# dusk-network/dusk-blindbidproof

Measured on AMD Instinct MI355X. Metric: blind-bid proofs/sec, higher is better.
Workload: dtype u32

## Files before the change

__graft_entry__.py:

```python
import os
import shutil
import subprocess
import sys

ROOT = os.path.dirname(os.path.abspath(__file__))
PKG = os.path.join(ROOT, "dusk_blindbidproof_amd")
CSRC = os.path.join(PKG, "csrc")
LIB = os.path.join(PKG, "libbbp_hip.so")
ORACLE_SO = os.path.join(ROOT, "oracle", "_build", "libbbp_oracle.so")
HOSTCHECK_SO = os.path.join(ROOT, "tests", "_build", "libhostcheck.so")
DEVCHECK_SO = {"chain": os.path.join(ROOT, "tests", "_build", "libbbp_devcheck.so"),
               "nochain": os.path.join(ROOT, "tests", "_build", "libbbp_devcheck_nochain.so")}
DEVCHECK_DEFS = {"chain": [], "nochain": ["-DBBP_FE_NO_CHAIN"]}


def _newer(target, sources):
    if not os.path.exists(target):
        return True
    t = os.path.getmtime(target)
    return any(os.path.getmtime(s) > t for s in sources)


def _run(cmd):
    print("+", " ".join(cmd), flush=True)
# ... 177 lines not shown
VERIFY_PLAN_SAN_BIN = os.path.join(ROOT, "tests", "_build", "verify_plan_san")


def build_verify_plan_san(force=False):
    src = os.path.join(ROOT, "tests", "verify_plan_san.cpp")
    if force or _newer(VERIFY_PLAN_SAN_BIN, [src, os.path.join(ROOT, "tests", "host_check.cpp")] + _csrc_files((".h", ".inc"))):
        os.makedirs(os.path.dirname(VERIFY_PLAN_SAN_BIN), exist_ok=True)
        _run(["g++", "-O1", "-g", "-std=c++17", "-fsanitize=address,undefined", "-fno-sanitize-recover=all", "-o", VERIFY_PLAN_SAN_BIN, src])
    return VERIFY_PLAN_SAN_BIN


BATCH_LAYOUT_SAN_BIN = os.path.join(ROOT, "tests", "_build", "batch_layout_san")


def build_batch_layout_san(force=False):
    src = os.path.join(ROOT, "tests", "batch_layout_san.cpp")
    if force or _newer(BATCH_LAYOUT_SAN_BIN, [src, os.path.join(ROOT, "tests", "host_check.cpp")] + _csrc_files((".h", ".inc"))):
        os.makedirs(os.path.dirname(BATCH_LAYOUT_SAN_BIN), exist_ok=True)
        _run(["g++", "-O1", "-g", "-std=c++17", "-fsanitize=address,undefined", "-fno-sanitize-recover=all", "-o", BATCH_LAYOUT_SAN_BIN, src])
    return BATCH_LAYOUT_SAN_BIN


HEDGE_SAN_BIN = os.path.join(ROOT, "tests", "_build", "hedge_san")


def build_hedge_san(force=False):
    src = os.path.join(ROOT, "tests", "hedge_san.cpp")
    if force or _newer(HEDGE_SAN_BIN, [src] + _csrc_files((".h", ".inc"))):
        os.makedirs(os.path.dirname(HEDGE_SAN_BIN), exist_ok=True)
        _run(["g++", "-O1", "-g", "-std=c++17", "-fsanitize=address,undefined", "-fno-sanitize-recover=all", "-o", HEDGE_SAN_BIN, src])
    return HEDGE_SAN_BIN


SECRET_MAP_BIN = os.path.join(ROOT, "tests", "_build", "secret_map_check")
SECRET_WIPE_SAN_BIN = os.path.join(ROOT, "tests", "_build", "secret_wipe_san")


def build_secret_map_check(force=False):
    src = os.path.join(ROOT, "tests", "secret_map_check.cpp")
    if force or _newer(SECRET_MAP_BIN, [src] + _csrc_files((".h", ".inc"))):
        os.makedirs(os.path.dirname(SECRET_MAP_BIN), exist_ok=True)
        _run(["g++", "-O1", "-g", "-std=c++17", "-fsanitize=address,undefined", "-fno-sanitize-recover=all", "-o", SECRET_MAP_BIN, src])
    return SECRET_MAP_BIN


ROUND_SELECT_BIN = os.path.join(ROOT, "tests", "_build", "round_select_check")


def build_round_select_check(force=False):
    src = os.path.join(ROOT, "tests", "round_select_check.cpp")
    if force or _newer(ROUND_SELECT_BIN, [src] + _csrc_files((".h", ".inc")) + [os.path.join(ROOT, "include", "bbp.h")]):
        os.makedirs(os.path.dirname(ROUND_SELECT_BIN), exist_ok=True)
        _run(["g++", "-O1", "-g", "-std=c++17", "-fsanitize=address,undefined", "-fno-sanitize-recover=all", "-o", ROUND_SELECT_BIN, src])
    return ROUND_SELECT_BIN


ROUND_BEST_BIN = os.path.join(ROOT, "tests", "_build", "round_best_check")


def build_round_best_check(force=False):
    src = os.path.join(ROOT, "tests", "round_best_check.cpp")
    if force or _newer(ROUND_BEST_BIN, [src] + _csrc_files((".h", ".inc")) + [os.path.join(ROOT, "include", "bbp.h")]):
        os.makedirs(os.path.dirname(ROUND_BEST_BIN), exist_ok=True)
        _run(["g++", "-O1", "-g", "-std=c++17", "-fsanitize=address,undefined", "-fno-sanitize-recover=all", "-o", ROUND_BEST_BIN, src])
    return ROUND_BEST_BIN

# ... 105 lines not shown
        flags = ["-O1", "-g", "-fsanitize=thread"] if tsan else ["-O1"]
        _run(["g++"] + flags + ["-std=c++17", "-pthread", "-o", out] + srcs)
    return out


COMBINER_ROUNDS_BIN = {False: os.path.join(ROOT, "tests", "_build", "combiner_rounds"), True: os.path.join(ROOT, "tests", "_build", "combiner_rounds_tsan")}


def build_combiner_rounds(tsan=False, force=False):
    out = COMBINER_ROUNDS_BIN[bool(tsan)]
    srcs = [os.path.join(ROOT, "tests", "combiner_rounds.cpp"), os.path.join(CSRC, "submit.cpp")]
    if force or _newer(out, srcs + [os.path.join(CSRC, "submit.h")]):
        os.makedirs(os.path.dirname(out), exist_ok=True)
        flags = ["-O1", "-g", "-fsanitize=thread"] if tsan else ["-O1"]
        _run(["g++"] + flags + ["-std=c++17", "-pthread", "-o", out] + srcs)
    return out


def build():
    build_hip()
    build_server()
    build_stub_engine()
    build_oracle()
    build_hostcheck()
    build_sortcheck()
    build_roundcheck()
    build_round_select_check()
    build_round_best_check()
    build_round_best_distinct_check()
    build_rounds_best_check()
    build_rounds_best_distinct_check()
    build_round_standing_check()
    build_standings_check()
    build_devcheck_all()
    sys.path.insert(0, ROOT)
    import dusk_blindbidproof_amd


def smoke():
    sys.path.insert(0, ROOT)
    import dusk_blindbidproof_amd as bbp
    from tests import smoke_case

    smoke_case.run(bbp)


if __name__ == "__main__":
    build()
```

dusk_blindbidproof_amd/csrc/msm.hip:

```cpp
#include "context.h"

namespace bbp {

#ifndef BBP_FOLD_PRIO
#define BBP_FOLD_PRIO 2
#endif
#ifndef BBP_MSM_WAVES
#define BBP_MSM_WAVES 2
#endif
#ifndef BBP_MSM_WAVES_MAX
#define BBP_MSM_WAVES_MAX 2
#endif

#ifdef BBP_MSM_PROF
__device__ unsigned long long g_msm_prof[8];
#define MSM_PROF_BEGIN() unsigned long long prof_t = wall_clock64()
#define MSM_PROF_MARK(i)                                                    \
    if (tid == 0) {                                                         \
        unsigned long long now_ = wall_clock64();                           \
        atomicAdd(&g_msm_prof[i], now_ - prof_t);                           \
        prof_t = now_;                                                      \
    }
#else
#define MSM_PROF_BEGIN()
// ... 466 lines not shown
        ge acc = ge_identity();
        u32 ent_cur = sorted[c0];
        u32 ent_nxt = (c0 + 1 < c1) ? sorted[c0 + 1] : 0u;
        row_regs row = load_row(ptable, ent_cur, fault);
        for (u32 e = c0; e < c1; e++) {
            if (e == kend) {
                *dest = acc;
                acc = ge_identity();
                do { k++; kend = cursor[k]; } while (kend == e);
                dest = &bsum[k - 1];
            }
            const row_regs cur = row;
            const bool neg = ent_cur >> 31;
            ent_cur = ent_nxt;
            if (e + 1 < c1) row = load_row(ptable, ent_cur, fault);
            if (e + 2 < c1) ent_nxt = sorted[e + 2];
            acc = ge_madd_row(acc, cur, neg);
        }
        *dest = acc;
    }
#endif
#ifdef BBP_MSM_PROF
    if (tid == 0) atomicAdd(&g_msm_prof[6], clock64() - clk0);
#endif
    MSM_PROF_MARK(2);
    __threadfence_block();
    __syncthreads();
    MSM_PROF_MARK(3);
#ifdef BBP_ACC_PERSIST
  }
#endif
}

template <int MODE>
__global__ __launch_bounds__(MSM_T) void k_msm_fold(const u32* __restrict__ cursor_all, ge* __restrict__ bsum_all, const ge* __restrict__ psum_all,
                                                     ge* __restrict__ out, const u32* __restrict__ n_active) {
    constexpr int K = msm_geom<MODE>::K, G = K / MSM_T;
    __shared__ u32 cursor[K + 1];
    __shared__ u32 xch[GE_WORDS];
    const int tid = threadIdx.x;
    if (n_active && blockIdx.x >= *n_active) return;
    __builtin_amdgcn_s_setprio(BBP_FOLD_PRIO);
    const size_t msm = blockIdx.x;
    {
        const u32* cur_in = cursor_all + msm * (size_t)(K + 1);
        for (int k = tid; k <= K; k += MSM_T) cursor[k] = cur_in[k];
    }
    __syncthreads();
    const u32 E = cursor[K];
    ge* bsum = bsum_all + msm * (size_t)K;
    const ge* psum = psum_all + msm * (size_t)ACC_T;
#ifdef BBP_KO_FOLD
    if (MODE != 1) { if (tid == 0) out[msm] = bsum[0]; }
    else if (tid < FOLD_CLS) out[msm * FOLD_CLS + tid] = bsum[tid];
    return;
#endif
    for (u32 ch = tid; ch < (u32)ACC_T; ch += MSM_T) {
        const u32 c0 = (u32)(((u64)ch * E) / ACC_T), c1 = (u32)(((u64)(ch + 1) * E) / ACC_T);
        if (c0 >= c1) continue;
        u32 lo = 1, hi = K;
        while (lo < hi) {
            u32 mid = (lo + hi) >> 1;
            if (cursor[mid] > c0) hi = mid; else lo = mid + 1;
        }
        const u32 k_first = lo;
        const bool inside = cursor[lo - 1] < c0;
        const bool last_of_run = inside && !(c1 < E && c1 > cursor[k_first - 1] && c1 < cursor[k_first]);
        if (last_of_run) {
            ge part = psum[ch];
            for (int u = (int)ch - 1; u >= 0; u--) {
                const u32 cu = (u32)(((u64)u * E) / ACC_T), cu1 = (u32)(((u64)(u + 1) * E) / ACC_T);
                if (cu <= cursor[k_first - 1]) break;
                if (cu1 > cu) ge_add_nc(part, part, psum[u]);
            }
            ge head = bsum[k_first - 1];
            ge_add_nc(head, head, part);
            bsum[k_first - 1] = head;
        }
    }
    __threadfence_block();
    __syncthreads();

    ge running = ge_identity(), total = ge_identity();
    if constexpr (G == 1) {
        if (cursor[tid + 1] != cursor[tid]) running = bsum[tid];
        total = running;
    } else {
#pragma unroll 1
        for (int r = G; r >= 1; r--) {
            const u32 k = tid * G + r;
            if (cursor[k] != cursor[k - 1]) running = ge_add(running, bsum[k - 1]);
            total = ge_add(total, running);
        }
    }

    if constexpr (MODE != 1) {
        const int lane = tid & 63, wave = tid >> 6;
#pragma unroll 1
        for (int d = 1; d < 64; d <<= 1) {
            ge other = ge_shfl_down(running, d);
            if (lane + d < 64) running = ge_add(running, other);
        }
        if (MSM_T > 64) {
            if (tid == 64) xch_put(xch, running);
            __syncthreads();
            if (wave == 0) {
                ge other = xch_get(xch);
                ge_add_nc(running, running, other);
            }
        }
        ge x = total;
        if (tid >= 1) {
            ge s = running;
            constexpr int LOG_G = G == 1 ? 0 : G == 2 ? 1 : G == 4 ? 2 : G == 8 ? 3 : G == 16 ? 4 : -1;
            static_assert(LOG_G >= 0, "buckets per fold lane must be a power of two up to 16");
            for (int i = 0; i < LOG_G; i++) ge_dbl_nc(s, s);
            ge_add_nc(x, x, s);
        }
#pragma unroll 1
        for (int d = 32; d >= 1; d >>= 1) {
            ge other = ge_shfl_down(x, d);
            if (lane < d) x = ge_add(x, other);
        }
        if (MSM_T > 64) {
            __syncthreads();
            if (tid == 64) xch_put(xch, x);
            __syncthreads();
        }
        if (tid == 0) {
            if (MSM_T > 64) {
                ge other = xch_get(xch);
                ge_add_nc(x, x, other);
            }
            ge other;
            ge_dbl_nc(x, x);
            other = ge_neg(running);
            ge_add_nc(x, x, other);
            out[msm] = x;
        }
    } else {
        constexpr int LPC = FOLD_M / G, LOG_G2 = G == 32 ? 5 : 6;
        static_assert(G == 32 || G == 64, "class reduction written for 4 or 2 lanes per class");
        const int q = tid & (LPC - 1);
        ge suf = running;
        for (int d = 1; d < LPC; d++) {
            ge other = ge_shfl_down(running, d);
            if (q + d < LPC) ge_add_nc(suf, suf, other);
        }
        ge x = total;
        if (q >= 1) {
            ge sg = suf;
            for (int i = 0; i < LOG_G2; i++) ge_dbl_nc(sg, sg);
            ge_add_nc(x, x, sg);
        }
        ge accq = x;
        for (int d = 1; d < LPC; d++) {
            ge other = ge_shfl_down(x, d);
            if (q == 0) ge_add_nc(accq, accq, other);
        }
        if (q == 0) {
            ge_dbl_nc(accq, accq);
            ge other = ge_neg(suf);
            ge_add_nc(accq, accq, other);
            out[msm * FOLD_CLS + (tid / LPC)] = accq;
        }
    }
}

constexpr int FOLD2_L = 32;
constexpr int FOLD2_G = MSM_K / FOLD2_L;
constexpr int FOLD2_LOG_G = 5;
static_assert(FOLD2_G == 32 && ACC_T % FOLD2_L == 0, "fold geometry");

__device__ __forceinline__ ge ge_shfl_down32(const ge& p, int d) {
    ge r;
    const u32* w = reinterpret_cast<const u32*>(&p);
    u32* o = reinterpret_cast<u32*>(&r);
#pragma unroll
    for (int i = 0; i < GE_WORDS; i++) o[i] = (u32)__shfl_down((int)w[i], d, 32);
    return r;
}

__device__ __forceinline__ ge ge_add_t2d(const ge& p, const fe& p2d, const ge& q) {
    fe a = fe_mul(fe_sub(p.Y, p.X), fe_sub(q.Y, q.X));
    fe b = fe_mul(fe_add(p.Y, p.X), fe_add(q.Y, q.X));
    fe c = fe_mul(p2d, q.T);
    fe zz = fe_mul(p.Z, q.Z);
    fe d = fe_add(zz, zz);
    fe e = fe_sub(b, a), f = fe_sub(d, c), g = fe_add(d, c), h = fe_add(b, a);
    ge r;
    r.X = fe_mul(e, f);
    r.Y = fe_mul(g, h);
    r.Z = fe_mul(g, f);
    r.T = fe_mul(e, h);
    return r;
}

__device__ __forceinline__ void park_put(u32* park, int tid, const ge& p) {
    const u32* w = reinterpret_cast<const u32*>(&p);
#pragma unroll
    for (int i = 0; i < GE_WORDS; i++) park[i * 64 + tid] = w[i];
}

__device__ __forceinline__ ge park_get(const u32* park, int tid) {
    ge p;
    u32* w = reinterpret_cast<u32*>(&p);
#pragma unroll
    for (int i = 0; i < GE_WORDS; i++) w[i] = park[i * 64 + tid];
    return p;
}

__device__ __forceinline__ ge ld_ge(const ge* p) {
    ge r;
    const uint4* s = reinterpret_cast<const uint4*>(p);
    u32* o = reinterpret_cast<u32*>(&r);
#pragma unroll
    for (int i = 0; i < GE_WORDS / 4; i++) {
        const uint4 v = s[i];
        o[4 * i] = v.x, o[4 * i + 1] = v.y, o[4 * i + 2] = v.z, o[4 * i + 3] = v.w;
    }
    return r;
}

#ifndef BBP_FOLD_WAVES
#define BBP_FOLD_WAVES 2
#endif
__global__ __launch_bounds__(64) __attribute__((amdgpu_waves_per_eu(BBP_FOLD_WAVES, BBP_FOLD_WAVES))) void k_msm_fold_half(const u32* __restrict__ cursor_all, ge* __restrict__ bsum_all, const ge* __restrict__ psum_all,
                                                       ge* __restrict__ out, u32 n_work, const u32* __restrict__ n_active) {
    constexpr int K = MSM_K, G = FOLD2_G;
    __shared__ u32 cursor2[2][K + 1];
    __shared__ u32 park[GE_WORDS * 64];
    const int tid = threadIdx.x, half = tid >> 5, l = tid & 31;
    const u32 n_tot = n_active ? min(*n_active, n_work) : n_work;
    if (2u * blockIdx.x >= n_tot) return;
    __builtin_amdgcn_s_setprio(BBP_FOLD_PRIO);
    const size_t msm = 2 * (size_t)blockIdx.x + half;
    const bool valid = msm < n_tot;
    u32* cursor = cursor2[half];
    {
        const u32* cur_in = cursor_all + msm * (size_t)(K + 1);
        for (int k = l; k <= K; k += FOLD2_L) cursor[k] = valid ? cur_in[k] : 0u;
    }
    __syncthreads();
    const u32 E = cursor[K];
    ge* bsum = bsum_all + (valid ? msm : 0) * (size_t)K;
    const ge* psum = psum_all + (valid ? msm : 0) * (size_t)ACC_T;
#pragma unroll 1
    for (u32 ch = l; ch < (u32)ACC_T; ch += FOLD2_L) {
        const u32 c0 = (u32)(((u64)ch * E) / ACC_T), c1 = (u32)(((u64)(ch + 1) * E) / ACC_T);
        bool last_of_run = false;
        u32 k_first = 1;
        if (c0 < c1) {
            u32 lo = 1, hi = K;
            while (lo < hi) {
// ... 319 lines not shown
```

dusk_blindbidproof_amd/csrc/prover.hip:

```cpp
#define BBP_KECCAK_WAVE 1
#include <string.h>

#include <functional>

#include "batch.h"
#include "hosthash.h"
#include "keccak_wave.h"
#include "scalarmul.h"
#include "witness.h"

namespace bbp {

#define BBP_THIN_PRIO() __builtin_amdgcn_s_setprio(3)
#ifndef BBP_LANE_KERNEL
#define BBP_LANE_KERNEL __launch_bounds__(64)
#endif


__device__ __forceinline__ void sc_to_bytes32(uint8_t* o, const sc& s) { sc_tobytes(o, s); }
__device__ __forceinline__ void words_to_bytes32(uint8_t* o, const u32* w) {
#pragma unroll
    for (int i = 0; i < 8; i++) {
        o[4 * i] = (uint8_t)w[i];
        o[4 * i + 1] = (uint8_t)(w[i] >> 8);
// ... 848 lines not shown
}

__global__ __launch_bounds__(64) __attribute__((amdgpu_waves_per_eu(2, 3))) void k_tail_tables(u32 count, const ge* __restrict__ pts, ge* __restrict__ tab) {
    BBP_THIN_PRIO();
    u32 t = blockIdx.x * blockDim.x + threadIdx.x;
    if (t >= count) return;
    ge P = pts[t];
    ge* T = tab + (size_t)t * TAIL_TAB;
#pragma unroll 1
    for (int k = 0; k < TAIL_PIECES; k++) {
        ge cur = P;
        T[8 * k] = P;
#pragma unroll 1
        for (int i = 1; i < 8; i++) {
            cur = ge_add(cur, P);
            T[8 * k + i] = cur;
        }
        if (k < TAIL_PIECES - 1) {
#pragma unroll 1
            for (int i = 0; i < TAIL_PIECE_BITS; i++) P = ge_dbl(P);
        }
    }
}

__global__ void k_tail_init(u32 B, sc* __restrict__ g_all, sc* __restrict__ h_all) {
    BBP_THIN_PRIO();
    u32 t = blockIdx.x * blockDim.x + threadIdx.x;
    if (t >= B * FOLD_CLS) return;
    const u32 p = t / FOLD_CLS, k = t % FOLD_CLS;
    st_sc(&g_all[(size_t)p * IPA_N + k], sc_one());
    st_sc(&h_all[(size_t)p * IPA_N + k], sc_one());
}

#ifndef BBP_TAIL_SPLIT
#define BBP_TAIL_SPLIT 1
#endif
#ifndef BBP_TAIL_MERGE
#define BBP_TAIL_MERGE 1
#endif
#ifndef BBP_TAIL_BLK
#define BBP_TAIL_BLK (BBP_TAIL_SPLIT == 1 ? 256 : 320)
#endif
constexpr int TAIL_SPLIT = BBP_TAIL_SPLIT, TAIL_MERGE = BBP_TAIL_MERGE, TAIL_LS = TAIL_MERGE == 2 ? 17 : 33 * TAIL_SPLIT, TAIL_BLK = BBP_TAIL_BLK, TAIL_LP = 2 * TAIL_LS, TAIL_PPB = TAIL_BLK / TAIL_LP;
static_assert(TAIL_PIECES % TAIL_SPLIT == 0 && TAIL_PPB >= 1 && (TAIL_MERGE == 1 || (TAIL_MERGE == 2 && TAIL_SPLIT == 1)), "tail kernel geometry");
__global__ __launch_bounds__(TAIL_BLK) void k_tail_lr(u32 B, u32 n, u32 prev_round, u32 m, const u32* __restrict__ enc, merlin_transcript* __restrict__ tr,
                                                       const sc* __restrict__ misc, sc* __restrict__ a_all, sc* __restrict__ b_all,
                                                       sc* __restrict__ g_all, sc* __restrict__ h_all, const ge* __restrict__ ftab,
                                                       const ge* __restrict__ btab, ge* __restrict__ lrpts) {
    BBP_THIN_PRIO();
    __shared__ u32 stage[GE_WORDS * TAIL_BLK];
    __shared__ u32 uu_w[TAIL_PPB * 2 * 8];
    const u32 tid = threadIdx.x;
    const u32 pj = tid / TAIL_LP, l = tid % TAIL_LP;
    const u32 p = blockIdx.x * TAIL_PPB + pj;
    const bool live = pj < TAIL_PPB && p < B;
    const u32 side = l / TAIL_LS, rem = l % TAIL_LS;
    const u32 j = TAIL_MERGE == 2 ? 2 * rem : rem / TAIL_SPLIT, share = rem % TAIL_SPLIT;
    const size_t po = live ? (size_t)p : 0;
    sc *a = a_all + po * IPA_N, *b = b_all + po * IPA_N, *gg = g_all + po * IPA_N, *hh = h_all + po * IPA_N;
    if (prev_round) {
        if (live && l == 0) {
            merlin_transcript t = tr[p];
            const u32* e = enc + (size_t)p * enc_words(m) + enc_LR(m, prev_round);
            tr_append_words(t, LBL("L"), e);
            tr_append_words(t, LBL("R"), e + 8);
            const sc u = tr_challenge_sc(t, LBL("u")), ui = sc_invert(u);
#pragma unroll
            for (int w = 0; w < 8; w++) {
                uu_w[(pj * 2) * 8 + w] = u.v[w];
                uu_w[(pj * 2 + 1) * 8 + w] = ui.v[w];
            }
            tr[p] = t;
        }
        __syncthreads();
        if (live) {
            sc u, ui;
#pragma unroll
            for (int w = 0; w < 8; w++) {
                u.v[w] = uu_w[(pj * 2) * 8 + w];
                ui.v[w] = uu_w[(pj * 2 + 1) * 8 + w];
            }
            const u32 n2 = 2 * n;
            for (u32 w = l; w < 2 * n2 + 2 * FOLD_CLS; w += TAIL_LP) {
                if (w < n2) {
                    st_sc(&a[w], sc_add(sc_mul(ld_sc(&a[w]), u), sc_mul(ui, ld_sc(&a[n2 + w]))));
                } else if (w < 2 * n2) {
                    const u32 i = w - n2;
                    st_sc(&b[i], sc_add(sc_mul(ld_sc(&b[i]), ui), sc_mul(u, ld_sc(&b[n2 + i]))));
                } else {
                    const u32 k = (w - 2 * n2) % FOLD_CLS;
                    const bool hi = (k & (2 * n2 - 1)) >= n2;
                    if (w - 2 * n2 < FOLD_CLS) st_sc(&gg[k], sc_mul(ld_sc(&gg[k]), hi ? u : ui));
                    else st_sc(&hh[k], sc_mul(ld_sc(&hh[k]), hi ? ui : u));
                }
            }
        }
        __threadfence_block();
        __syncthreads();
    }
    const ge *FG = ftab + po * 2 * FOLD_CLS * TAIL_TAB, *FH = FG + (size_t)FOLD_CLS * TAIL_TAB;
    constexpr u32 HALF = FOLD_CLS / 2;
    auto term = [&](u32 jt, sc& s, const ge*& T) {
        if (jt < 2 * HALF) {
            const u32 rank = jt % HALF, blk = rank / n, io = rank % n;
            const u32 k_lo = blk * 2 * n + io, k_hi = k_lo + n;
            if (jt < HALF) {
                const u32 k = side == 0 ? k_hi : k_lo;
                s = sc_mul(ld_sc(&a[side == 0 ? io : n + io]), ld_sc(&gg[k]));
                T = FG + (size_t)k * TAIL_TAB;
            } else {
                const u32 k = side == 0 ? k_lo : k_hi;
                s = sc_mul(ld_sc(&b[side == 0 ? n + io : io]), ld_sc(&hh[k]));
                T = FH + (size_t)k * TAIL_TAB;
            }
        } else {
            sc c = sc_zero();
            for (u32 i = 0; i < n; i++)
                c = sc_add(c, side == 0 ? sc_mul(ld_sc(&a[i]), ld_sc(&b[n + i])) : sc_mul(ld_sc(&a[n + i]), ld_sc(&b[i])));
            s = sc_mul(c, ld_sc(&misc[(size_t)p * MS_COUNT + MS_W]));
            T = btab;
        }
    };
    ge q = ge_identity();
    if (live) {
        sc s;
        const ge* T;
        term(j, s, T);
#ifndef BBP_KO_TAIL
        if (TAIL_MERGE == 2 && j + 1 < 2 * HALF + 1) {
            sc s2;
            const ge* T2;
            term(j + 1, s2, T2);
            q = ge_scalarmul_pieces_pair(s, T, s2, T2);
        } else {
            constexpr int PPS = TAIL_PIECES / TAIL_SPLIT;
            q = ge_scalarmul_pieces(s, T, (int)share * PPS, (int)share * PPS + PPS);
        }
#else
        q = T[0];
        q.X.v[0] += (i32)(s.v[0] & 1u);
#endif
    }
    const u32* w = reinterpret_cast<const u32*>(&q);
    for (int k = 0; k < GE_WORDS; k++) stage[k * TAIL_BLK + tid] = w[k];
    __syncthreads();
    for (int d = 64; d >= 1; d >>= 1) {
        if (live && rem < (u32)d && rem + d < (u32)TAIL_LS) {
            ge o;
            u32* ow = reinterpret_cast<u32*>(&o);
            for (int k = 0; k < GE_WORDS; k++) ow[k] = stage[k * TAIL_BLK + tid + d];
            q = ge_add(q, o);
            for (int k = 0; k < GE_WORDS; k++) stage[k * TAIL_BLK + tid] = reinterpret_cast<const u32*>(&q)[k];
        }
        __syncthreads();
    }
    if (live && rem == 0) lrpts[(size_t)p * 2 + side] = q;
}

__global__ BBP_LANE_KERNEL void k_ipa_final(u32 B, u32 m, const u32* __restrict__ enc, merlin_transcript* __restrict__ tr, sc* __restrict__ misc,
                            const sc* __restrict__ a_all, const sc* __restrict__ b_all, u32 wave) {
    BBP_THIN_PRIO();
    u32 p = blockIdx.x * blockDim.x + threadIdx.x;
    if (wave) p >>= 6;
    if (p >= B) return;
    merlin_transcript t = tr[p];
    t.wave = wave;
    const u32* e = enc + (size_t)p * enc_words(m) + enc_LR(m, IPA_ROUNDS);
    tr_append_words(t, LBL("L"), e);
    tr_append_words(t, LBL("R"), e + 8);
    sc u = tr_challenge_sc(t, LBL("u"));
    sc ui = sc_invert(u);
    const sc *a = a_all + (size_t)p * IPA_N, *b = b_all + (size_t)p * IPA_N;
    sc* ms = misc + (size_t)p * MS_COUNT;
    st_sc(&ms[MS_A0], sc_add(sc_mul(ld_sc(&a[0]), u), sc_mul(ui, ld_sc(&a[1]))));
    st_sc(&ms[MS_B0], sc_add(sc_mul(ld_sc(&b[0]), ui), sc_mul(u, ld_sc(&b[1]))));
    t.wave = 0;
    tr[p] = t;
}

__global__ BBP_LANE_KERNEL void k_assemble(u32 B, u32 m, const u32* __restrict__ enc, const sc* __restrict__ misc, u8* __restrict__ out) {
    BBP_THIN_PRIO();
    u32 p = blockIdx.x * blockDim.x + threadIdx.x;
    if (p >= B) return;
    const u32* e = enc + (size_t)p * enc_words(m);
    const sc* ms = misc + (size_t)p * MS_COUNT;
    u8* o = out + (size_t)p * (BBP_R1CS_PROOF_BYTES + 32 * (size_t)m);
    *o++ = 0;
    auto put = [&](const u32* w) {
        words_to_bytes32(o, w);
// ... 129 lines not shown
           bd.wo, bd.wv, st.wl);
    LAUNCH(ctx, TAG_POLY, k_poly, B, POLY_BLK, s, n1, bd.ai1, bd.ao1, bd.s1, bd.wl, bd.wr, bd.wo, st.wl, bd.ypow, bd.yipow, bd.l1, bd.r0,
           bd.r1, bd.r3, bd.misc);
    LAUNCH(ctx, TAG_TRANSCRIPT, k_tr_tblind, tgrid, 64, s, B, bd.rng, bd.misc, tw);
    if (hp.split_T)
        LAUNCH(ctx, TAG_COMMIT, k_commit_T_split, cdiv(B * 5 * COMMIT_L, 64), 64, s, B, bd.misc, ctx->comb, bd.pts, st.pts, m);
    else
        LAUNCH(ctx, TAG_COMMIT, k_commit_T, cdiv(B * 5, 64), 64, s, B, bd.misc, ctx->comb, bd.pts, st.pts, m);
    LAUNCH(ctx, TAG_ENCODE, k_encode_strided, cdiv(B * 5, 64), 64, s, B * 5, 5u, bd.pts + pts_T(m), st.pts, bd.enc, st.enc, enc_T(m), 1u);
    LAUNCH(ctx, TAG_TRANSCRIPT, k_tr_ux, tgrid, 64, s, B, m, n1, bd.enc, bd.wv, bd.vb, bd.ai1, bd.ao1, bd.s1, bd.tr, bd.misc, tw);
    LAUNCH(ctx, TAG_POLY, k_lrvec, cdiv(B * IPA_N, 128), 128, s, B, n1, bd.l1, bd.r0, bd.r1, bd.r3, bd.ao1, bd.s1, bd.ypow, bd.yipow, bd.misc,
           bd.a, bd.b, bd.g, bd.h);
    const u32 tail_from = hp.tail_from;
    for (u32 r = 1; r <= IPA_ROUNDS && r < tail_from; r++) {
        if (r > 1) LAUNCH(ctx, TAG_TRANSCRIPT, k_ipa_challenge, tgrid, 64, s, B, r - 1, m, bd.enc, bd.tr, bd.misc, tw);
        if (hp.wide_ipa)
            LAUNCH(ctx, TAG_IPA_SCALARS, k_ipa_round<IPA_BLK_WIDE>, B, IPA_BLK_WIDE, s, r, n1, bd.misc, bd.a, bd.b, bd.g, bd.h, bd.lr);
        else
            LAUNCH(ctx, TAG_IPA_SCALARS, k_ipa_round<IPA_BLK>, B, IPA_BLK, s, r, n1, bd.misc, bd.a, bd.b, bd.g, bd.h, bd.lr);
        if ((rc = msm_launch(ctx, 2 * B, IPA_TERMS, (const u32*)bd.lr, c.idx_ipa + (size_t)(r - 1) * st.lr, bd.lrpts, s, 2, slot))) return rc;
        LAUNCH(ctx, TAG_ENCODE, k_encode_strided, cdiv(2 * B, 64), 64, s, 2 * B, 2u, bd.lrpts, st.lrpts, bd.enc, st.enc, enc_LR(m, r), 1u);
    }
    if (tail_from <= IPA_ROUNDS) {
        DevBuf& vt = ctx->slice_vtab[slot];
        if ((rc = dev_reserve(ctx, vt, (size_t)B * 2 * FOLD_CLS * TAIL_TAB * sizeof(ge)))) return rc;
        ge* ftab = static_cast<ge*>(vt.p);
        LAUNCH(ctx, TAG_TRANSCRIPT, k_ipa_challenge, tgrid, 64, s, B, tail_from - 1, m, bd.enc, bd.tr, bd.misc, tw);
        LAUNCH(ctx, TAG_IPA_SCALARS, k_ipa_round<IPA_BLK>, B, IPA_BLK, s, tail_from, n1, bd.misc, bd.a, bd.b, bd.g, bd.h, (sc*)nullptr);
        if ((rc = fold_generators_launch(ctx, B, bd.g, bd.h, bd.fpts, s, slot))) return rc;
        LAUNCH(ctx, TAG_VARBASE, k_tail_init, cdiv(B * FOLD_CLS, 64), 64, s, B, bd.g, bd.h);
        LAUNCH(ctx, TAG_VARBASE, k_tail_tables, cdiv(B * 2 * FOLD_CLS, 64), 64, s, B * 2 * FOLD_CLS, bd.fpts, ftab);
        for (u32 r = tail_from; r <= IPA_ROUNDS; r++) {
            const u32 n = IPA_HALF >> (r - 1);
            LAUNCH(ctx, TAG_VARBASE, k_tail_lr, cdiv(B, TAIL_PPB), TAIL_BLK, s, B, n, r > tail_from ? r - 1 : 0u, m, bd.enc, bd.tr, bd.misc, bd.a, bd.b, bd.g, bd.h, ftab,
                   ctx->btab, bd.lrpts);
            LAUNCH(ctx, TAG_ENCODE, k_encode_strided, cdiv(2 * B, 64), 64, s, 2 * B, 2u, bd.lrpts, st.lrpts, bd.enc, st.enc, enc_LR(m, r), 1u);
        }
    }
    LAUNCH(ctx, TAG_TRANSCRIPT, k_ipa_final, tgrid, 64, s, B, m, bd.enc, bd.tr, bd.misc, bd.a, bd.b, tw);
    if (out_guard) BBP_HIP_TRY(ctx, hipStreamWaitEvent(s, out_guard, 0));
    LAUNCH(ctx, TAG_TRANSCRIPT, k_assemble, cdiv(B, 64), 64, s, B, m, bd.enc, bd.misc, out_dev);
    if (wipe_on(ctx)) {
        WipeList wl;
        wipe_take(wl, ptsbuf);
        wipe_take(wl, slot ? ctx->slice_sorted[slot] : ctx->sorted);
        wipe_take(wl, ctx->slice_fold[slot]);
        wipe_take(wl, ctx->slice_vtab[slot]);
        if ((rc = wipe_enqueue(ctx, wl, s))) return rc;
    }
    return BBP_OK;
}

int32_t prove_batch_dev(bbp_ctx* ctx, u32 B, u32 N, const u8* in_dev, const u8* ent_dev, u8* out_dev, hipStream_t s,
                        const std::function<int32_t(hipStream_t)>* open_hook) {
    const CircuitDev* cp;
    int32_t rc = circuit_get(ctx, N, &cp);
    if (rc) return rc;
    const CircuitDev& c = *cp;
    StreamGuard guard(ctx, s);
    if ((rc = guard.enter())) return rc;
    int inflight = 0;
    for (int k = 0; k < bbp_ctx::CALL_RING; k++)
        if (ctx->ev_call_valid[k] && hipEventQuery(ctx->ev_call[k]) == hipErrorNotReady) inflight++;
    const ProvePlan plan = plan_prove(ctx->knobs, ctx->prove_state, B, inflight, [&] {
        const int lp = ctx->last_prove_par;
        return lp >= 0 && ctx->ev_done_valid[lp] && hipEventQuery(ctx->ev_done[lp]) == hipErrorNotReady;
    });
// ... 118 lines not shown
```

dusk_blindbidproof_amd/csrc/scalarmul.h:

```cpp
#pragma once
#include "point.h"
#include "scalar.h"

namespace bbp {

#if defined(__HIPCC__)
#define BBP_COMB_LOAD(n, entry)                                                                  \
    do {                                                                                         \
        const uint4* q_ = reinterpret_cast<const uint4*>(entry);                                 \
        uint4 q0 = q_[0], q1 = q_[1], q2 = q_[2], q3 = q_[3], q4 = q_[4], q5 = q_[5];            \
        (n).ypx = BBP_FE_LIT(q0.x, q0.y, q0.z, q0.w, q1.x, q1.y, q1.z, q1.w);                    \
        (n).ymx = BBP_FE_LIT(q2.x, q2.y, q2.z, q2.w, q3.x, q3.y, q3.z, q3.w);                    \
        (n).xy2d = BBP_FE_LIT(q4.x, q4.y, q4.z, q4.w, q5.x, q5.y, q5.z, q5.w);                   \
    } while (0)
#else
#define BBP_COMB_LOAD(n, entry)                     \
    do {                                            \
        const u32* w_ = (entry)->w;                 \
        (n).ypx = fe_fromwords(w_);                 \
        (n).ymx = fe_fromwords(w_ + 8);             \
        (n).xy2d = fe_fromwords(w_ + 16);           \
    } while (0)
#endif

// ... 140 lines not shown
        c1 = v1 > 8u;
        c2 = v2 > 8u;
        if (j < 63) {
            cm1 |= (u64)c1 << (j + 1);
            cm2 |= (u64)c2 << (j + 1);
        }
    }
    ge acc = ge_identity();
    for (int r = TAIL_DIGITS - 1; r >= 0; r--) {
        if (r != TAIL_DIGITS - 1) {
            acc = ge_dbl(acc);
            acc = ge_dbl(acc);
            acc = ge_dbl(acc);
            acc = ge_dbl(acc);
        }
#pragma unroll 1
        for (int kk = 0; kk < 2 * TAIL_PIECES; kk++) {
            const int k = kk >> 1;
            const bool second = kk & 1;
            const int j = TAIL_DIGITS * k + r;
            const u32 word = second ? s2.v[j >> 3] : s1.v[j >> 3];
            const u64 cm = second ? cm2 : cm1;
            const int d = (int)((word >> (4 * (j & 7))) & 15u) + (int)((cm >> j) & 1u) - 16 * (int)((j < 63) ? ((cm >> (j + 1)) & 1u) : 0u);
            if (d != 0) {
                ge q = (second ? T2 : T1)[8 * k + (d > 0 ? d : -d) - 1];
                if (d < 0) q = ge_neg(q);
                acc = ge_add(acc, q);
            }
        }
    }
    return acc;
}

BBP_HD void straus_recode(u32* sp, const sc& s) {
    u64 cy = 0;
#pragma unroll
    for (int i = 0; i < 8; i++) {
        cy += (u64)s.v[i] + 0x88888888u;
        sp[i] = (u32)cy;
        cy >>= 32;
    }
}

BBP_HD void straus_table(ge* tab, const ge& P) {
    tab[0] = P;
    ge cur = P;
    for (int i = 1; i < 8; i++) {
        cur = ge_add(cur, P);
        tab[i] = cur;
    }
}

template <class J>
BBP_HD ge straus_digit_step(ge acc, const ge* tab, const u32* sp, J j) {
    const int d = (int)((sp[j >> 3] >> (4 * (j & 7))) & 15u) - 8;
    if (d != 0) {
        ge e = tab[(d > 0 ? d : -d) - 1];
        if (d < 0) e = ge_neg(e);
        acc = ge_add(acc, e);
    }
    return acc;
}

}
```

Baseline: 23140.

## Restructure tail L/R kernel to one wavefront per proof with shared B-term digits

Measured after the change: 23440 (median of 6 runs). 1.3% higher.

```diff
diff --git a/__graft_entry__.py b/__graft_entry__.py
--- a/__graft_entry__.py
+++ b/__graft_entry__.py
@@ -233,6 +233,18 @@
     return HEDGE_SAN_BIN
 
 
+TAIL_SHARE_BIN = os.path.join(ROOT, "tests", "_build", "tail_share_check")
+
+
+def build_tail_share_check(force=False):
+    src = os.path.join(ROOT, "tests", "tail_share_check.cpp")
+    if force or _newer(TAIL_SHARE_BIN, [src] + _csrc_files((".h", ".inc"))):
+        os.makedirs(os.path.dirname(TAIL_SHARE_BIN), exist_ok=True)
+        _run(["g++", "-O1", "-g", "-std=c++17", "-fsanitize=address,undefined", "-fno-sanitize=signed-integer-overflow,shift", "-fno-sanitize-recover=all", "-o",
+              TAIL_SHARE_BIN, src])
+    return TAIL_SHARE_BIN
+
+
 SECRET_MAP_BIN = os.path.join(ROOT, "tests", "_build", "secret_map_check")
 SECRET_WIPE_SAN_BIN = os.path.join(ROOT, "tests", "_build", "secret_wipe_san")
 
@@ -404,6 +416,7 @@
     build_rounds_best_distinct_check()
     build_round_standing_check()
     build_standings_check()
+    build_tail_share_check()
     build_devcheck_all()
     sys.path.insert(0, ROOT)
     import dusk_blindbidproof_amd
diff --git a/dusk_blindbidproof_amd/csrc/msm.hip b/dusk_blindbidproof_amd/csrc/msm.hip
--- a/dusk_blindbidproof_amd/csrc/msm.hip
+++ b/dusk_blindbidproof_amd/csrc/msm.hip
@@ -522,6 +522,33 @@
 #endif
 }
 
+__device__ __forceinline__ ge ge_add_t2d(const ge& p, const fe& p2d, const ge& q) {
+    fe a = fe_mul(fe_sub(p.Y, p.X), fe_sub(q.Y, q.X));
+    fe b = fe_mul(fe_add(p.Y, p.X), fe_add(q.Y, q.X));
+    fe c = fe_mul(p2d, q.T);
+    fe zz = fe_mul(p.Z, q.Z);
+    fe d = fe_add(zz, zz);
+    fe e = fe_sub(b, a), f = fe_sub(d, c), g = fe_add(d, c), h = fe_add(b, a);
+    ge r;
+    r.X = fe_mul(e, f);
+    r.Y = fe_mul(g, h);
+    r.Z = fe_mul(g, f);
+    r.T = fe_mul(e, h);
+    return r;
+}
+
+__device__ __forceinline__ ge ld_ge(const ge* p) {
+    ge r;
+    const uint4* s = reinterpret_cast<const uint4*>(p);
+    u32* o = reinterpret_cast<u32*>(&r);
+#pragma unroll
+    for (int i = 0; i < GE_WORDS / 4; i++) {
+        const uint4 v = s[i];
+        o[4 * i] = v.x, o[4 * i + 1] = v.y, o[4 * i + 2] = v.z, o[4 * i + 3] = v.w;
+    }
+    return r;
+}
+
 template <int MODE>
 __global__ __launch_bounds__(MSM_T) void k_msm_fold(const u32* __restrict__ cursor_all, ge* __restrict__ bsum_all, const ge* __restrict__ psum_all,
                                                      ge* __restrict__ out, const u32* __restrict__ n_active) {
@@ -557,15 +584,29 @@
         const bool inside = cursor[lo - 1] < c0;
         const bool last_of_run = inside && !(c1 < E && c1 > cursor[k_first - 1] && c1 < cursor[k_first]);
         if (last_of_run) {
-            ge part = psum[ch];
-            for (int u = (int)ch - 1; u >= 0; u--) {
-                const u32 cu = (u32)(((u64)u * E) / ACC_T), cu1 = (u32)(((u64)(u + 1) * E) / ACC_T);
-                if (cu <= cursor[k_first - 1]) break;
-                if (cu1 > cu) ge_add_nc(part, part, psum[u]);
-            }
-            ge head = bsum[k_first - 1];
-            ge_add_nc(head, head, part);
-            bsum[k_first - 1] = head;
+            if constexpr (MODE == 1) {
+                ge part = ld_ge(&psum[ch]);
+                for (int u = (int)ch - 1; u >= 0; u--) {
+                    const u32 cu = (u32)(((u64)u * E) / ACC_T), cu1 = (u32)(((u64)(u + 1) * E) / ACC_T);
+                    if (cu <= cursor[k_first - 1]) break;
+                    if (cu1 > cu) {
+                        const ge more = ld_ge(&psum[u]);
+                        part = ge_add(part, more);
+                    }
+                }
+                const ge head = ld_ge(&bsum[k_first - 1]);
+                bsum[k_first - 1] = ge_add(head, part);
+            } else {
+                ge part = psum[ch];
+                for (int u = (int)ch - 1; u >= 0; u--) {
+                    const u32 cu = (u32)(((u64)u * E) / ACC_T), cu1 = (u32)(((u64)(u + 1) * E) / ACC_T);
+                    if (cu <= cursor[k_first - 1]) break;
+                    if (cu1 > cu) ge_add_nc(part, part, psum[u]);
+                }
+                ge head = bsum[k_first - 1];
+                ge_add_nc(head, head, part);
+                bsum[k_first - 1] = head;
+            }
         }
     }
     __threadfence_block();
@@ -575,6 +616,24 @@
     if constexpr (G == 1) {
         if (cursor[tid + 1] != cursor[tid]) running = bsum[tid];
         total = running;
+    } else if constexpr (MODE == 1) {
+        fe r2d = fe_zero();
+#pragma unroll 1
+        for (int st = 2 * G - 1; st >= 0; st--) {
+            const u32 k = tid * G + (u32)(st >> 1) + 1;
+            const bool into_total = !(st & 1);
+            if (into_total || cursor[k] != cursor[k - 1]) {
+                ge q = total;
+                if (!into_total) q = ld_ge(&bsum[k - 1]);
+                const ge sum = ge_add_t2d(running, r2d, q);
+                if (into_total) {
+                    total = sum;
+                } else {
+                    running = sum;
+                    r2d = fe_mul(running.T, fe_d2());
+                }
+            }
+        }
     } else {
 #pragma unroll 1
         for (int r = G; r >= 1; r--) {
@@ -631,29 +690,36 @@
     } else {
         constexpr int LPC = FOLD_M / G, LOG_G2 = G == 32 ? 5 : 6;
         static_assert(G == 32 || G == 64, "class reduction written for 4 or 2 lanes per class");
+        constexpr int LOG_LPC = LPC == 4 ? 2 : 1;
+        static_assert((1 << LOG_LPC) == LPC, "lanes per class");
         const int q = tid & (LPC - 1);
-        ge suf = running;
-        for (int d = 1; d < LPC; d++) {
-            ge other = ge_shfl_down(running, d);
-            if (q + d < LPC) ge_add_nc(suf, suf, other);
-        }
-        ge x = total;
-        if (q >= 1) {
-            ge sg = suf;
-            for (int i = 0; i < LOG_G2; i++) ge_dbl_nc(sg, sg);
-            ge_add_nc(x, x, sg);
-        }
-        ge accq = x;
-        for (int d = 1; d < LPC; d++) {
-            ge other = ge_shfl_down(x, d);
-            if (q == 0) ge_add_nc(accq, accq, other);
-        }
-        if (q == 0) {
-            ge_dbl_nc(accq, accq);
-            ge other = ge_neg(suf);
-            ge_add_nc(accq, accq, other);
-            out[msm * FOLD_CLS + (tid / LPC)] = accq;
-        }
+        ge v = running, keep = total;
+#pragma unroll 1
+        for (int it = 0; it < 2 * LOG_LPC + 2; it++) {
+            ge o;
+            bool take;
+            int n_dbl = 0;
+            if (it == LOG_LPC) {
+                o = v;
+                v = keep;
+                keep = o;
+                n_dbl = LOG_G2;
+                take = q >= 1;
+            } else if (it == 2 * LOG_LPC + 1) {
+                o = v;
+                v = ge_neg(keep);
+                n_dbl = 1;
+                take = true;
+            } else {
+                const int d = it < LOG_LPC ? (1 << it) : ((LPC / 2) >> (it - LOG_LPC - 1));
+                o = ge_shfl_down(v, d);
+                take = it < LOG_LPC ? (q + d < LPC) : (q < d);
+            }
+#pragma unroll 1
+            for (int i = 0; i < n_dbl; i++) o = ge_dbl(o);
+            if (take) v = ge_add(v, o);
+        }
+        if (q == 0) out[msm * FOLD_CLS + (tid / LPC)] = v;
     }
 }
 
@@ -671,21 +737,6 @@
     return r;
 }
 
-__device__ __forceinline__ ge ge_add_t2d(const ge& p, const fe& p2d, const ge& q) {
-    fe a = fe_mul(fe_sub(p.Y, p.X), fe_sub(q.Y, q.X));
-    fe b = fe_mul(fe_add(p.Y, p.X), fe_add(q.Y, q.X));
-    fe c = fe_mul(p2d, q.T);
-    fe zz = fe_mul(p.Z, q.Z);
-    fe d = fe_add(zz, zz);
-    fe e = fe_sub(b, a), f = fe_sub(d, c), g = fe_add(d, c), h = fe_add(b, a);
-    ge r;
-    r.X = fe_mul(e, f);
-    r.Y = fe_mul(g, h);
-    r.Z = fe_mul(g, f);
-    r.T = fe_mul(e, h);
-    return r;
-}
-
 __device__ __forceinline__ void park_put(u32* park, int tid, const ge& p) {
     const u32* w = reinterpret_cast<const u32*>(&p);
 #pragma unroll
@@ -698,18 +749,6 @@
 #pragma unroll
     for (int i = 0; i < GE_WORDS; i++) w[i] = park[i * 64 + tid];
     return p;
-}
-
-__device__ __forceinline__ ge ld_ge(const ge* p) {
-    ge r;
-    const uint4* s = reinterpret_cast<const uint4*>(p);
-    u32* o = reinterpret_cast<u32*>(&r);
-#pragma unroll
-    for (int i = 0; i < GE_WORDS / 4; i++) {
-        const uint4 v = s[i];
-        o[4 * i] = v.x, o[4 * i + 1] = v.y, o[4 * i + 2] = v.z, o[4 * i + 3] = v.w;
-    }
-    return r;
 }
 
 #ifndef BBP_FOLD_WAVES
diff --git a/dusk_blindbidproof_amd/csrc/prover.hip b/dusk_blindbidproof_amd/csrc/prover.hip
--- a/dusk_blindbidproof_amd/csrc/prover.hip
+++ b/dusk_blindbidproof_amd/csrc/prover.hip
@@ -904,129 +904,90 @@
     st_sc(&h_all[(size_t)p * IPA_N + k], sc_one());
 }
 
-#ifndef BBP_TAIL_SPLIT
-#define BBP_TAIL_SPLIT 1
-#endif
-#ifndef BBP_TAIL_MERGE
-#define BBP_TAIL_MERGE 1
-#endif
-#ifndef BBP_TAIL_BLK
-#define BBP_TAIL_BLK (BBP_TAIL_SPLIT == 1 ? 256 : 320)
-#endif
-constexpr int TAIL_SPLIT = BBP_TAIL_SPLIT, TAIL_MERGE = BBP_TAIL_MERGE, TAIL_LS = TAIL_MERGE == 2 ? 17 : 33 * TAIL_SPLIT, TAIL_BLK = BBP_TAIL_BLK, TAIL_LP = 2 * TAIL_LS, TAIL_PPB = TAIL_BLK / TAIL_LP;
-static_assert(TAIL_PIECES % TAIL_SPLIT == 0 && TAIL_PPB >= 1 && (TAIL_MERGE == 1 || (TAIL_MERGE == 2 && TAIL_SPLIT == 1)), "tail kernel geometry");
+__device__ __forceinline__ sc sc_shfl(const sc& s, int src) {
+    sc r;
+#pragma unroll
+    for (int w = 0; w < 8; w++) r.v[w] = (u32)__shfl((int)s.v[w], src, 64);
+    return r;
+}
+__device__ __forceinline__ sc sc_shfl_xor(const sc& s, int mask) {
+    sc r;
+#pragma unroll
+    for (int w = 0; w < 8; w++) r.v[w] = (u32)__shfl_xor((int)s.v[w], mask, 64);
+    return r;
+}
+constexpr int TAIL_BLK = 2 * TAIL_SIDE;
+static_assert(TAIL_BLK == 64 && TAIL_SIDE == FOLD_CLS, "k_tail_lr: one wavefront per proof, one lane per (side, G/H term)");
 __global__ __launch_bounds__(TAIL_BLK) void k_tail_lr(u32 B, u32 n, u32 prev_round, u32 m, const u32* __restrict__ enc, merlin_transcript* __restrict__ tr,
                                                        const sc* __restrict__ misc, sc* __restrict__ a_all, sc* __restrict__ b_all,
                                                        sc* __restrict__ g_all, sc* __restrict__ h_all, const ge* __restrict__ ftab,
                                                        const ge* __restrict__ btab, ge* __restrict__ lrpts) {
     BBP_THIN_PRIO();
-    __shared__ u32 stage[GE_WORDS * TAIL_BLK];
-    __shared__ u32 uu_w[TAIL_PPB * 2 * 8];
-    const u32 tid = threadIdx.x;
-    const u32 pj = tid / TAIL_LP, l = tid % TAIL_LP;
-    const u32 p = blockIdx.x * TAIL_PPB + pj;
-    const bool live = pj < TAIL_PPB && p < B;
-    const u32 side = l / TAIL_LS, rem = l % TAIL_LS;
-    const u32 j = TAIL_MERGE == 2 ? 2 * rem : rem / TAIL_SPLIT, share = rem % TAIL_SPLIT;
-    const size_t po = live ? (size_t)p : 0;
-    sc *a = a_all + po * IPA_N, *b = b_all + po * IPA_N, *gg = g_all + po * IPA_N, *hh = h_all + po * IPA_N;
+    const u32 p = blockIdx.x, l = threadIdx.x;
+    if (p >= B) return;
+    const u32 side = l / TAIL_SIDE, j = l % TAIL_SIDE;
+    sc *a = a_all + (size_t)p * IPA_N, *b = b_all + (size_t)p * IPA_N, *gg = g_all + (size_t)p * IPA_N, *hh = h_all + (size_t)p * IPA_N;
     if (prev_round) {
-        if (live && l == 0) {
-            merlin_transcript t = tr[p];
-            const u32* e = enc + (size_t)p * enc_words(m) + enc_LR(m, prev_round);
-            tr_append_words(t, LBL("L"), e);
-            tr_append_words(t, LBL("R"), e + 8);
-            const sc u = tr_challenge_sc(t, LBL("u")), ui = sc_invert(u);
-#pragma unroll
-            for (int w = 0; w < 8; w++) {
-                uu_w[(pj * 2) * 8 + w] = u.v[w];
-                uu_w[(pj * 2 + 1) * 8 + w] = ui.v[w];
+        merlin_transcript t = tr[p];
+        t.wave = 1;
+        const u32* e = enc + (size_t)p * enc_words(m) + enc_LR(m, prev_round);
+        tr_append_words(t, LBL("L"), e);
+        tr_append_words(t, LBL("R"), e + 8);
+        const sc u = tr_challenge_sc(t, LBL("u"));
+        sc ui = sc_zero();
+        if (l == 0) {
+            ui = sc_invert(u);
+            t.wave = 0;
+            tr[p] = t;
+        }
+        ui = sc_shfl(ui, 0);
+        const u32 n2 = 2 * n;
+        for (u32 w = l; w < 2 * n2 + 2 * FOLD_CLS; w += TAIL_BLK) {
+            if (w < n2) {
+                st_sc(&a[w], sc_add(sc_mul(ld_sc(&a[w]), u), sc_mul(ui, ld_sc(&a[n2 + w]))));
+            } else if (w < 2 * n2) {
+                const u32 i = w - n2;
+                st_sc(&b[i], sc_add(sc_mul(ld_sc(&b[i]), ui), sc_mul(u, ld_sc(&b[n2 + i]))));
+            } else {
+                const u32 k = (w - 2 * n2) % FOLD_CLS;
+                const bool hi = (k & (2 * n2 - 1)) >= n2;
+                if (w - 2 * n2 < FOLD_CLS) st_sc(&gg[k], sc_mul(ld_sc(&gg[k]), hi ? u : ui));
+                else st_sc(&hh[k], sc_mul(ld_sc(&hh[k]), hi ? ui : u));
             }
-            tr[p] = t;
-        }
-        __syncthreads();
-        if (live) {
-            sc u, ui;
-#pragma unroll
-            for (int w = 0; w < 8; w++) {
-                u.v[w] = uu_w[(pj * 2) * 8 + w];
-                ui.v[w] = uu_w[(pj * 2 + 1) * 8 + w];
-            }
-            const u32 n2 = 2 * n;
-            for (u32 w = l; w < 2 * n2 + 2 * FOLD_CLS; w += TAIL_LP) {
-                if (w < n2) {
-                    st_sc(&a[w], sc_add(sc_mul(ld_sc(&a[w]), u), sc_mul(ui, ld_sc(&a[n2 + w]))));
-                } else if (w < 2 * n2) {
-                    const u32 i = w - n2;
-                    st_sc(&b[i], sc_add(sc_mul(ld_sc(&b[i]), ui), sc_mul(u, ld_sc(&b[n2 + i]))));
-                } else {
-                    const u32 k = (w - 2 * n2) % FOLD_CLS;
-                    const bool hi = (k & (2 * n2 - 1)) >= n2;
-                    if (w - 2 * n2 < FOLD_CLS) st_sc(&gg[k], sc_mul(ld_sc(&gg[k]), hi ? u : ui));
-                    else st_sc(&hh[k], sc_mul(ld_sc(&hh[k]), hi ? ui : u));
-                }
-            }
         }
         __threadfence_block();
-        __syncthreads();
-    }
-    const ge *FG = ftab + po * 2 * FOLD_CLS * TAIL_TAB, *FH = FG + (size_t)FOLD_CLS * TAIL_TAB;
+        __builtin_amdgcn_wave_barrier();
+    }
+    const ge *FG = ftab + (size_t)p * 2 * FOLD_CLS * TAIL_TAB, *FH = FG + (size_t)FOLD_CLS * TAIL_TAB;
     constexpr u32 HALF = FOLD_CLS / 2;
-    auto term = [&](u32 jt, sc& s, const ge*& T) {
-        if (jt < 2 * HALF) {
-            const u32 rank = jt % HALF, blk = rank / n, io = rank % n;
-            const u32 k_lo = blk * 2 * n + io, k_hi = k_lo + n;
-            if (jt < HALF) {
-                const u32 k = side == 0 ? k_hi : k_lo;
-                s = sc_mul(ld_sc(&a[side == 0 ? io : n + io]), ld_sc(&gg[k]));
-                T = FG + (size_t)k * TAIL_TAB;
-            } else {
-                const u32 k = side == 0 ? k_lo : k_hi;
-                s = sc_mul(ld_sc(&b[side == 0 ? n + io : io]), ld_sc(&hh[k]));
-                T = FH + (size_t)k * TAIL_TAB;
-            }
+    sc s;
+    const ge* T;
+    {
+        const u32 rank = j % HALF, blk = rank / n, io = rank % n;
+        const u32 k_lo = blk * 2 * n + io, k_hi = k_lo + n;
+        if (j < HALF) {
+            const u32 k = side == 0 ? k_hi : k_lo;
+            s = sc_mul(ld_sc(&a[side == 0 ? io : n + io]), ld_sc(&gg[k]));
+            T = FG + (size_t)k * TAIL_TAB;
         } else {
-            sc c = sc_zero();
-            for (u32 i = 0; i < n; i++)
-                c = sc_add(c, side == 0 ? sc_mul(ld_sc(&a[i]), ld_sc(&b[n + i])) : sc_mul(ld_sc(&a[n + i]), ld_sc(&b[i])));
-            s = sc_mul(c, ld_sc(&misc[(size_t)p * MS_COUNT + MS_W]));
-            T = btab;
-        }
-    };
-    ge q = ge_identity();
-    if (live) {
-        sc s;
-        const ge* T;
-        term(j, s, T);
+            const u32 k = side == 0 ? k_lo : k_hi;
+            s = sc_mul(ld_sc(&b[side == 0 ? n + io : io]), ld_sc(&hh[k]));
+            T = FH + (size_t)k * TAIL_TAB;
+        }
+    }
+    sc c = sc_zero();
+    if (j < n) c = side == 0 ? sc_mul(ld_sc(&a[j]), ld_sc(&b[n + j])) : sc_mul(ld_sc(&a[n + j]), ld_sc(&b[j]));
+#pragma unroll 1
+    for (int d = TAIL_SIDE / 2; d >= 1; d >>= 1) c = sc_add(c, sc_shfl_xor(c, d));
+    const sc sB = sc_mul(c, ld_sc(&misc[(size_t)p * MS_COUNT + MS_W]));
 #ifndef BBP_KO_TAIL
-        if (TAIL_MERGE == 2 && j + 1 < 2 * HALF + 1) {
-            sc s2;
-            const ge* T2;
-            term(j + 1, s2, T2);
-            q = ge_scalarmul_pieces_pair(s, T, s2, T2);
-        } else {
-            constexpr int PPS = TAIL_PIECES / TAIL_SPLIT;
-            q = ge_scalarmul_pieces(s, T, (int)share * PPS, (int)share * PPS + PPS);
-        }
+    ge q = ge_scalarmul_pieces_shared(s, T, tail_share_of(sB, j), btab);
 #else
-        q = T[0];
-        q.X.v[0] += (i32)(s.v[0] & 1u);
+    ge q = T[0];
+    q.X.v[0] += (i32)((s.v[0] ^ sB.v[0]) & 1u);
 #endif
-    }
-    const u32* w = reinterpret_cast<const u32*>(&q);
-    for (int k = 0; k < GE_WORDS; k++) stage[k * TAIL_BLK + tid] = w[k];
-    __syncthreads();
-    for (int d = 64; d >= 1; d >>= 1) {
-        if (live && rem < (u32)d && rem + d < (u32)TAIL_LS) {
-            ge o;
-            u32* ow = reinterpret_cast<u32*>(&o);
-            for (int k = 0; k < GE_WORDS; k++) ow[k] = stage[k * TAIL_BLK + tid + d];
-            q = ge_add(q, o);
-            for (int k = 0; k < GE_WORDS; k++) stage[k * TAIL_BLK + tid] = reinterpret_cast<const u32*>(&q)[k];
-        }
-        __syncthreads();
-    }
-    if (live && rem == 0) lrpts[(size_t)p * 2 + side] = q;
+    q = tail_side_sum(q);
+    if (j == 0) lrpts[(size_t)p * 2 + side] = q;
 }
 
 __global__ BBP_LANE_KERNEL void k_ipa_final(u32 B, u32 m, const u32* __restrict__ enc, merlin_transcript* __restrict__ tr, sc* __restrict__ misc,
@@ -1222,7 +1183,7 @@
         LAUNCH(ctx, TAG_VARBASE, k_tail_tables, cdiv(B * 2 * FOLD_CLS, 64), 64, s, B * 2 * FOLD_CLS, bd.fpts, ftab);
         for (u32 r = tail_from; r <= IPA_ROUNDS; r++) {
             const u32 n = IPA_HALF >> (r - 1);
-            LAUNCH(ctx, TAG_VARBASE, k_tail_lr, cdiv(B, TAIL_PPB), TAIL_BLK, s, B, n, r > tail_from ? r - 1 : 0u, m, bd.enc, bd.tr, bd.misc, bd.a, bd.b, bd.g, bd.h, ftab,
+            LAUNCH(ctx, TAG_VARBASE, k_tail_lr, B, TAIL_BLK, s, B, n, r > tail_from ? r - 1 : 0u, m, bd.enc, bd.tr, bd.misc, bd.a, bd.b, bd.g, bd.h, ftab,
                    ctx->btab, bd.lrpts);
             LAUNCH(ctx, TAG_ENCODE, k_encode_strided, cdiv(2 * B, 64), 64, s, 2 * B, 2u, bd.lrpts, st.lrpts, bd.enc, st.enc, enc_LR(m, r), 1u);
         }
diff --git a/dusk_blindbidproof_amd/csrc/scalarmul.h b/dusk_blindbidproof_amd/csrc/scalarmul.h
--- a/dusk_blindbidproof_amd/csrc/scalarmul.h
+++ b/dusk_blindbidproof_amd/csrc/scalarmul.h
@@ -196,6 +196,85 @@
     return acc;
 }
 
+constexpr int TAIL_SIDE = 32, TAIL_SHARE_DIGITS = TAIL_PIECES * TAIL_DIGITS / TAIL_SIDE;
+static_assert(TAIL_SHARE_DIGITS >= 1 && TAIL_SHARE_DIGITS * TAIL_SIDE == TAIL_PIECES * TAIL_DIGITS && TAIL_DIGITS % TAIL_SHARE_DIGITS == 0 &&
+                  (TAIL_DIGITS / TAIL_SHARE_DIGITS) * TAIL_PIECES == TAIL_SIDE,
+              "the shares of the B term tile its digits: every (piece, digit) belongs to exactly one lane of the side");
+
+BBP_HD u64 tail_carry_mask(const sc& s) {
+    u64 cm = 0;
+    u32 c = 0;
+    for (int j = 0; j < 64; j++) {
+        u32 v = ((s.v[j >> 3] >> (4 * (j & 7))) & 15u) + c;
+        c = v > 8u;
+        if (j < 63) cm |= (u64)c << (j + 1);
+    }
+    return cm;
+}
+BBP_HD int tail_digit(const sc& s, u64 cm, int j) {
+    u32 word = s.v[0];
+#pragma unroll
+    for (int w = 1; w < 8; w++) word = (j >> 3) == w ? s.v[w] : word;
+    return (int)((word >> (4 * (j & 7))) & 15u) +(int)((cm >> j) & 1u) - 16 * (int)((j < 63) ? ((cm >> (j + 1)) & 1u) : 0u);
+}
+
+struct tail_share {
+    int k, r0;
+    int d[TAIL_SHARE_DIGITS];
+};
+BBP_HD tail_share tail_share_of(const sc& sB, u32 lane ) {
+    const u64 cm = tail_carry_mask(sB);
+    tail_share sh;
+    sh.k = (int)(lane % TAIL_PIECES);
+    sh.r0 = TAIL_SHARE_DIGITS * (int)(lane / TAIL_PIECES);
+    for (int i = 0; i < TAIL_SHARE_DIGITS; i++) sh.d[i] = tail_digit(sB, cm, TAIL_DIGITS * sh.k + sh.r0 + i);
+    return sh;
+}
+
+BBP_HD ge ge_scalarmul_pieces_shared(const sc& s, const ge* __restrict__ T, const tail_share& sh, const ge* __restrict__ TB) {
+    const u64 cm = tail_carry_mask(s);
+    ge acc = ge_identity();
+    for (int r = TAIL_DIGITS - 1; r >= 0; r--) {
+        if (r != TAIL_DIGITS - 1) {
+            acc = ge_dbl(acc);
+            acc = ge_dbl(acc);
+            acc = ge_dbl(acc);
+            acc = ge_dbl(acc);
+        }
+        const int i = r - sh.r0;
+        const bool mine = i >= 0 && i < TAIL_SHARE_DIGITS;
+        int dB = 0;
+        for (int q = 0; q < TAIL_SHARE_DIGITS; q++) dB = q == i ? sh.d[q] : dB;
+#pragma unroll 1
+        for (int kk = 0; kk < TAIL_PIECES + 1; kk++) {
+            const bool own = kk < TAIL_PIECES;
+            if (!own && !mine) break;
+            const int k = own ? kk : sh.k;
+            const int d = own ? tail_digit(s, cm, TAIL_DIGITS * k + r) : dB;
+            if (d != 0) {
+                ge q = (own ? T : TB)[8 * k + (d > 0 ? d : -d) - 1];
+                if (d < 0) q = ge_neg(q);
+                acc = ge_add(acc, q);
+            }
+        }
+    }
+    return acc;
+}
+#if defined(__HIPCC__)
+__device__ __forceinline__ ge tail_side_sum(ge acc) {
+#pragma unroll 1
+    for (int d = TAIL_SIDE / 2; d >= 1; d >>= 1) {
+        ge other;
+        const u32* w = reinterpret_cast<const u32*>(&acc);
+        u32* o = reinterpret_cast<u32*>(&other);
+#pragma unroll
+        for (int i = 0; i < (int)(sizeof(ge) / 4); i++) o[i] = (u32)__shfl_down((int)w[i], d, TAIL_SIDE);
+        acc = ge_add(acc, other);
+    }
+    return acc;
+}
+#endif
+
 BBP_HD void straus_recode(u32* sp, const sc& s) {
     u64 cy = 0;
 #pragma unroll
```
